# Zokrates/ZoKrates

Hardware: AMD Instinct MI355X
Metric: groth16_proofs_per_sec (higher is better)
Workload: dtype u32

## Files before the change

zokrates_amd/csrc/core.cuh:

```cuda
#pragma once
#include <algorithm>
#include <atomic>
#include <chrono>
#include <cstdio>
#include <memory>
#include <new>
#include <string>
#include <system_error>
#include <thread>
#include <unordered_set>
#include <vector>

#include "../../include/zkhip.h"
#include "devrt.h"
#include "ec.cuh"
#include "kernels_msm.cuh"
#include "kernels_ntt.cuh"

namespace zk {

struct CurveBn254 {
    static constexpr int ID = ZKHIP_CURVE_BN128;
    typedef Fe<Bn254Fr> Fr;
    typedef Fe<Bn254Fq> Fq;
// ... 53 lines not shown
template <class T> static inline T* ptr(const DBuf& b) { return (T*)b.p; }

static inline unsigned blocks_for(u64 n, unsigned threads) { return (unsigned)((n + threads - 1) / threads); }
static inline int ilog2_floor(u64 x) { int l = 0; while (x >>= 1) ++l; return l; }
static inline int ilog2_ceil(u64 x) { int l = 0; while (((u64)1 << l) < x) ++l; return l; }

}

using namespace zk;

struct NttPlanBase {
    int curve, logN;
    virtual ~NttPlanBase() {}
};
struct MsmSort {
    DBuf dig, sorted, cnt, off, cursor, chunk_sum, grand;
    DBuf pairs, ccur, tile_off;
    Event ready = nullptr;
};
struct MsmLane {
    Stream stream = 0;
    bool made = false;
    bool high_priority = false;
    DBuf lane_key, heavy, partial, bucket, rows, cols;
    Event done = nullptr;
    Stream fold_stream = 0;
    bool fold_made = false;
    bool fold_owned = true;
    Event acc_done = nullptr;
    bool lone_launch = false;
    Stream lone_fold_stream = 0;
    bool lone_fold_made = false;
    bool share_cu = false;
};
static constexpr int ZK_NLANES = 5;
static constexpr int ZK_NSLOTS = 4;
struct ProofSlot {
    DBuf scalars, zmont, va, vb, vc, ws1, ws2, zflag;
    MsmSort sorts[3];
    MsmLane lanes[ZK_NLANES];
    void* h_ws = nullptr;
    size_t h_ws_cap = 0;
    Event ev[4] = {nullptr, nullptr, nullptr, nullptr};
    Event acc_b[ZK_NLANES] = {}, acc_e[ZK_NLANES] = {};
    Event ntt_b = nullptr, ntt_e = nullptr;
    Event g1_go = nullptr;
    Event half_ready = nullptr;
// ... 385 lines not shown
static void ntt_kind_b(zkhip_ctx* ctx, NttPlan<C>* pl, typename C::Fr* data, bool inverse, const typename C::Fr* final_post, int nvec = 1,
                       u64 vec_stride = 0, int canon = 0) {
    typedef typename C::Fr Fr;
    if (pl->log3 > 0) {
        ntt_rows<C>(ctx, pl, data, inverse, inverse ? ptr<Fr>(pl->tw2_inv) : ptr<Fr>(pl->tw2_fwd), nvec, vec_stride, 0, nullptr, pl->Nb - 1);
        ntt_mid<C>(ctx, pl, data, inverse, inverse ? ptr<Fr>(pl->tw_inv) : ptr<Fr>(pl->tw_fwd), ~(u64)0, nvec, vec_stride);
        ntt_cols<C>(ctx, pl, data, inverse, final_post, nvec, vec_stride, canon);
    } else if (pl->log1 > 0) {
        ntt_rows<C>(ctx, pl, data, inverse, inverse ? ptr<Fr>(pl->tw_inv) : ptr<Fr>(pl->tw_fwd), nvec, vec_stride);
        ntt_cols<C>(ctx, pl, data, inverse, final_post, nvec, vec_stride, canon);
    } else {
        ntt_rows<C>(ctx, pl, data, inverse, final_post, nvec, vec_stride, canon);
    }
}

struct MsmShape {
    u64 n;
    int c, W;
    u32 K;
    u32 sets;
    u32 levels;
    u32 nkeys;
    u32 Lw, H;
    static constexpr u32 ndig = 2;
    int level_bits() const { return c * (int)sets; }
    bool skip_inf = true;
    u32 nsums() const { return ndig * sets; }
};
static inline int env_int(const char* name, int lo, int hi, int dflt) {
    if (const char* e = getenv(name)) { int v = atoi(e); if (v >= lo && v <= hi) return v; }
    return dflt;
}
static constexpr int MSM_MAX_C = 17;
static constexpr int MSM_AUTO_MAX_C = 17;
static constexpr int MSM_ADHOC_MAX_C = 16;
static constexpr u32 MSM_SORT_MAX_KH = 1u << 15;
static inline MsmShape msm_shape(const zkhip_ctx* ctx, u64 n, int scalar_bits, bool table, int force_c = 0, int force_sets = 0) {
    MsmShape s;
    s.n = n;
    const int lg = ilog2_floor(std::max<u64>(n, 1));
    if (table) {
        const int cmax = std::max(2, std::min(MSM_AUTO_MAX_C, lg + 1));
        const int Wmin = (scalar_bits + 1 + cmax - 1) / cmax;
        s.c = cmax;
        while (s.c > 2 && (scalar_bits + 1 + (s.c - 1) - 1) / (s.c - 1) == Wmin) --s.c;
    } else {
        const int want = std::max(2, std::min(MSM_ADHOC_MAX_C, lg - 5));
// ... 1605 lines not shown
```

zokrates_amd/csrc/devrt.h:

```cpp
#pragma once
#include <algorithm>
#include <atomic>
#include <cstddef>
#include <mutex>
#include <unordered_map>
#include <cstdint>
#include <cstdio>
#include <cstdlib>
#include <cstring>
#include <string>
#include <system_error>
#include <thread>
#include <vector>

#ifdef ZK_EMU
#include "emu.h"
#else
#include <hip/hip_runtime.h>
#endif

namespace zk {

struct DevError {
    std::string msg;
// ... 376 lines not shown
inline bool trace_enabled() {
    static const bool on = getenv("ZKHIP_TRACE") != nullptr;
    return on;
}
inline bool grid_nonempty(const dim3& g) { return g.x != 0 && g.y != 0 && g.z != 0; }
#define ZK_LAUNCH(kernel, grid, block, smem, stream, ...)                                 \
    do {                                                                                  \
        if (!zk::grid_nonempty(dim3(grid))) break;                                        \
        if (zk::trace_enabled()) fprintf(stderr, "[zkhip] launch %s ...", #kernel);       \
        zk::jitter_before(stream);                                                        \
        hipLaunchKernelGGL(kernel, grid, block, smem, stream, __VA_ARGS__);               \
        zk::dev_check_last();                                                             \
        if (zk::trace_enabled()) {                                                        \
            ZK_HIP_CHECK(hipStreamSynchronize(stream));                                   \
            fprintf(stderr, " done\n");                                                   \
        }                                                                                 \
    } while (0)
#define ZK_DYN_SMEM(name) extern __shared__ __attribute__((aligned(16))) unsigned char name[]
#ifndef ZK_WAVE_PRIO
#define ZK_WAVE_PRIO 3
#endif
#define ZK_PRIO_HIGH() __builtin_amdgcn_s_setprio(ZK_WAVE_PRIO)
#define ZK_WAVE_ANY(pred) (__builtin_amdgcn_ballot_w64(pred) != 0)
#ifdef ZK_CHECKED
#define ZK_ASSERT_IDX(cond) do { if (!(cond)) __builtin_trap(); } while (0)
#else
#define ZK_ASSERT_IDX(cond) ((void)0)
#endif

#else

typedef int Stream;
typedef double* Event;
inline int dev_count() { return 1; }
inline void dev_set(int) {}
inline void dev_pci_bus_id(int, char* out, size_t cap) { snprintf(out, cap, "0000:00:00.0"); }
inline void* dev_alloc(size_t bytes) { return aligned_alloc(256, ((bytes ? bytes : 16) + 255) / 256 * 256); }
inline void dev_free(void* p) { free(p); }
inline void* host_alloc_pinned(size_t bytes) { return dev_alloc(bytes); }
inline void host_free_pinned(void* p) { free(p); }
inline void dev_h2d(void* d, const void* h, size_t n, Stream) { memcpy(d, h, n); }
template <class Fill>
inline void dev_h2d_fill(void* d, size_t n, size_t unit, Stream, Fill&& fill, unsigned = 8) {
    const size_t units = n / unit, cut = units / 3 * unit;
    if (cut) fill((char*)d, (size_t)0, cut);
    if (n > cut) fill((char*)d + cut, cut, n - cut);
// ... 7 lines not shown
inline void dev_memset(void* d, int v, size_t n, Stream) { memset(d, v, n); }
inline Stream stream_create() { return 0; }
inline Stream stream_create_high_priority() { return 0; }
inline Stream stream_create_low_priority() { return 0; }
inline void stream_destroy(Stream) {}
inline void stream_sync(Stream) {}
inline void dev_sync_all() {}
inline void dev_mem_info(size_t* free_b, size_t* total_b) { *free_b = *total_b = (size_t)1 << 40; }
inline Event event_create() { return new double(0); }
inline void event_destroy(Event e) { delete e; }
inline void event_record(Event e, Stream) { *e = emu::now_ms(); }
inline void event_sync(Event) {}
inline void stream_wait_event(Stream, Event) {}
inline float event_elapsed_ms(Event a, Event b) { return (float)(*b - *a); }
inline void dev_check_last() {}
struct JitterState { std::atomic<int> max_us{0}; };
inline JitterState& jitter_state() { static JitterState st; return st; }

#define ZK_LAUNCH(kernel, grid, block, smem, stream, ...) \
    emu::launch(dim3(grid), dim3(block), (size_t)(smem), [&]() { kernel(__VA_ARGS__); })
#define ZK_DYN_SMEM(name) unsigned char* name = emu::dyn_smem()
#define ZK_PRIO_HIGH() ((void)0)
#define ZK_WAVE_ANY(pred) (pred)
#ifdef ZK_CHECKED
#define ZK_ASSERT_IDX(cond) do { if (!(cond)) { fprintf(stderr, "ZK_ASSERT_IDX failed: %s (%s:%d)\n", #cond, __FILE__, __LINE__); abort(); } } while (0)
#else
#define ZK_ASSERT_IDX(cond) ((void)0)
#endif

#endif

}
```

zokrates_amd/csrc/group.cuh:

```cuda
#pragma once
#include "core.cuh"
#include "bind.cuh"

namespace zk {

template <class FS>
void points_to_packed(zkhip_ctx* ctx, const Aff<FS>* d_in, void* d_out, u64 n) {
    typedef typename Unsat<FS>::type U;
    ZK_LAUNCH((k_points_to_packed<FS, U>), dim3(blocks_for(n, 256)), dim3(256), 0, ctx->stream, d_in, (AffPacked<U>*)d_out, n);
}

template <class FS>
void msm_table_levels(zkhip_ctx* ctx, void* d_table, u64 count, int c, int W) {
    typedef typename Unsat<FS>::type F;
    if (W <= 1 || count == 0) return;
    const u64 chunk = std::min<u64>(count, std::max<u64>(1024, ((u64)768 << 20) / ((u64)(W - 1) * (sizeof(Xyzz<F>) + sizeof(F)))));
    DBuf tmp, pre;
    tmp.ensure((u64)(W - 1) * chunk * sizeof(Xyzz<F>));
    pre.ensure((u64)(W - 1) * chunk * sizeof(F));
    for (u64 i0 = 0; i0 < count; i0 += chunk) {
        const u64 cnt = std::min(chunk, count - i0);
        ZK_LAUNCH((k_msm_table_levels<F, FS>), dim3(blocks_for(cnt, 256)), dim3(256), 0, ctx->stream, (AffPacked<F>*)d_table, count, i0, cnt, c, W,
                  ptr<Xyzz<F>>(tmp), ptr<F>(pre));
    }
    stream_sync(ctx->stream);
}

template <class FS>
void msm_run_tables(zkhip_ctx* ctx, MsmLane& lane, const MsmSort& so, const void* const* d_tables, int nt, const MsmShape& sh, Xyzz<FS>* d_window_sums,
                    u32 sum_stride, Event ev_begin, Event ev_end, Event accum_after, Xyzz<FS>* h_window_sums) {
    typedef typename Unsat<FS>::type F;
    require(nt >= 1 && nt <= MSM_MAX_TABLES, ZKHIP_ERR_BAD_ARG, "internal: number of tables of one MSM launch");
    MsmTables tables{};
    for (int t = 0; t < nt; ++t) tables.p[t] = d_tables[t];
    Stream s = ctx->serial ? ctx->stream : lane_stream(lane);
    stream_wait_event(s, so.ready);
    const int single = MsmTuning<F>::IS_EXT ? (ctx->msm_g2_waves ? ctx->msm_g2_waves : MsmTuning<F>::SLICE_WPE)
                                            : (ctx->msm_g1_waves ? ctx->msm_g1_waves : MsmTuning<F>::SLICE_WPE);
    const int wpe = ctx->msm_waves ? ctx->msm_waves : (nt > 1 ? std::max(1, (ctx->msm_fused_waves ? ctx->msm_fused_waves : MsmTuning<F>::FUSED_WPE)) : single);
    const u64 machine = ctx->msm_lanes ? (u64)ctx->msm_lanes : (u64)ctx->cus * 4 * 64 * wpe / (nt > 1 && !ctx->msm_waves ? nt : 1);
    const u32 nlanes = (u32)std::max<u64>(1, std::min<u64>(machine, (sh.n * (u64)sh.W + ctx->msm_min_slice - 1) / ctx->msm_min_slice));
    const bool share = lane.share_cu && !ctx->serial;
    lane.share_cu = false;
    const bool lone_launch = lane.lone_launch;
    lane.lone_launch = false;
    const MsmCut cut{nlanes, ctx->msm_min_slice, (u32)std::min<u64>(sh.n * (u64)sh.levels, 0x7fffffffu), share ? 1u : 0u};
    const u64 partial_stride = (u64)sh.nkeys + nlanes;
    lane.heavy.ensure(((size_t)sh.nkeys + 1) * 4);
    lane.lane_key.ensure((size_t)nlanes * 4);
    lane.partial.ensure((size_t)nt * partial_stride * sizeof(Xyzz<F>));
    lane.bucket.ensure((size_t)nt * sh.nkeys * sizeof(Xyzz<F>));
    lane.rows.ensure((size_t)nt * sh.sets * sh.H * sizeof(Xyzz<F>));
    lane.cols.ensure((size_t)nt * sh.sets * sh.Lw * sizeof(Xyzz<F>));
    lds_opt_in(ctx, (const void*)k_msm_fold_rows<F>);
    lds_opt_in(ctx, (const void*)k_msm_fold_cols<F>);
    lds_opt_in(ctx, (const void*)k_msm_fold_final<F, FS>);
    lds_opt_in(ctx, (const void*)k_msm_fold_final_scan<F, FS>);
    const unsigned T = 256;
    ZK_LAUNCH(k_msm_lane_keys, dim3(blocks_for(nlanes, T)), dim3(T), 0, s, ptr<u32>(so.off), sh.nkeys, cut, ptr<u32>(lane.lane_key), ptr<u32>(lane.heavy));
    ZK_LAUNCH(k_msm_find_heavy, dim3(blocks_for(sh.nkeys, T)), dim3(T), 0, s, ptr<u32>(so.off), sh.nkeys, cut, ptr<u32>(lane.heavy) + 1,
              ptr<u32>(lane.heavy));
    if (accum_after && !ctx->serial) stream_wait_event(s, accum_after);
    if (ev_begin) event_record(ev_begin, s);
    const size_t acc_lds = share ? std::max<size_t>(msm_accum_lds_bytes<F>(), (size_t)84 * 1024) : msm_accum_lds_bytes<F>();
    if (ctx->skip_inf_mode == 1 || (ctx->skip_inf_mode == 0 && sh.skip_inf)) {
        if (acc_lds > 64 * 1024) lds_opt_in(ctx, (const void*)k_msm_accum<F, MsmTuning<F>::ACCUM_WPE, true>);
        ZK_LAUNCH((k_msm_accum<F, MsmTuning<F>::ACCUM_WPE, true>), dim3(blocks_for(nlanes, T), nt), dim3(T), acc_lds, s, tables, ptr<u32>(so.off), ptr<u32>(so.sorted),
                  ptr<u32>(lane.lane_key), ptr<Xyzz<F>>(lane.partial), partial_stride, sh.nkeys, cut);
    } else {
        if (acc_lds > 64 * 1024) lds_opt_in(ctx, (const void*)k_msm_accum<F, MsmTuning<F>::ACCUM_WPE, false>);
        ZK_LAUNCH((k_msm_accum<F, MsmTuning<F>::ACCUM_WPE, false>), dim3(blocks_for(nlanes, T), nt), dim3(T), acc_lds, s, tables, ptr<u32>(so.off), ptr<u32>(so.sorted),
                  ptr<u32>(lane.lane_key), ptr<Xyzz<F>>(lane.partial), partial_stride, sh.nkeys, cut);
    }
    if (ev_end) event_record(ev_end, s);
    const bool lone_hop = lone_launch && (lane.lone_fold_made || (MsmTuning<F>::IS_EXT && lane.fold_made));
    if (!ctx->serial && (lone_launch ? lone_hop : (lane.fold_made || ctx->fold_hop == 1 || (ctx->fold_hop == 2 && MsmTuning<F>::IS_EXT)))) {
        event_record(lane.acc_done, s);
        s = (lone_launch && lane.lone_fold_made) ? lane.lone_fold_stream : lane_fold_stream(lane);
        stream_wait_event(s, lane.acc_done);
    }
    if (ctx->heavy_runs) {
        lds_opt_in(ctx, (const void*)k_msm_heavy_reduce<F>);
        const unsigned TH = (unsigned)ctx->heavy_threads;
        ZK_LAUNCH((k_msm_heavy_reduce<F>), dim3(MSM_HEAVY_CHUNKS, nt), dim3(TH), (size_t)TH * sizeof(Xyzz<F>), s, ptr<Xyzz<F>>(lane.partial), partial_stride,
                  ptr<u32>(so.off), sh.nkeys, cut, ptr<u32>(lane.heavy) + 1, ptr<u32>(lane.heavy));
    }
    FoldDigits digs{};
    const u32 widest = std::max(sh.H, sh.Lw);
    if ((ctx->fold_lines == 1 || (ctx->fold_lines == 2 && nt == 1)) && widest <= 256) {
        const unsigned TL = std::max<u32>(64, widest);
        lds_opt_in(ctx, (const void*)k_msm_fold_lines<F>);
        ZK_LAUNCH((k_msm_fold_lines<F>), dim3(widest, sh.sets * 2, nt), dim3(TL), (size_t)TL * sizeof(Xyzz<F>), s, ptr<Xyzz<F>>(lane.partial), partial_stride,
                  ptr<u32>(so.off), sh.nkeys, cut, sh.K, sh.Lw, sh.H, ptr<u32>(lane.heavy) + 1, ptr<u32>(lane.heavy), ctx->heavy_runs ? 1u : 0u,
                  ptr<Xyzz<F>>(lane.rows), ptr<Xyzz<F>>(lane.cols));
    } else {
        ZK_LAUNCH((k_msm_fold_rows<F>), dim3(sh.H, sh.sets, nt), dim3(sh.Lw), (size_t)sh.Lw * sizeof(Xyzz<F>), s, ptr<Xyzz<F>>(lane.partial), partial_stride,
                  ptr<u32>(so.off), sh.nkeys, cut, sh.K, sh.Lw, ptr<u32>(lane.heavy) + 1, ptr<u32>(lane.heavy), ctx->heavy_runs ? 1u : 0u, ptr<Xyzz<F>>(lane.bucket),
                  ptr<Xyzz<F>>(lane.rows));
        const u32 RG = sh.H;
        const u32 HG = std::max<u32>(1, std::min<u32>((u32)ctx->fold_hg, RG)), CW = std::min<u32>(sh.Lw, 256 / HG), NG = sh.H / RG;
        ZK_LAUNCH((k_msm_fold_cols<F>), dim3(sh.Lw / CW, sh.sets * NG, nt), dim3(CW, HG), (size_t)CW * HG * sizeof(Xyzz<F>), s, ptr<Xyzz<F>>(lane.bucket), (u64)sh.K,
                  (u64)sh.nkeys, sh.Lw, sh.H, RG, ptr<Xyzz<F>>(lane.cols));
    }
    digs.d[0] = FoldDigit{lane.cols.p, sh.Lw, 1, 0};
    digs.d[1] = FoldDigit{lane.rows.p, sh.H, 0, (u32)ilog2_floor(sh.Lw)};
    u32 longest = 0;
    for (u32 d = 0; d < sh.ndig; ++d) longest = std::max(longest, digs.d[d].len);
    const unsigned TS = std::max<u32>(64, longest);
    if (ctx->fold_scan && TS <= 256) {
        ZK_LAUNCH((k_msm_fold_final_scan<F, FS>), dim3(sh.sets, nt, sh.ndig), dim3(TS), TS * sizeof(Xyzz<F>), s, digs, d_window_sums, sum_stride);
    } else {
        const unsigned TF = std::max<u32>(64, sh.Lw);
        ZK_LAUNCH((k_msm_fold_final<F, FS>), dim3(sh.sets, nt), dim3(TF), TF * sizeof(Xyzz<F>), s, ptr<Xyzz<F>>(lane.rows), ptr<Xyzz<F>>(lane.cols), sh.Lw,
                  sh.H, d_window_sums, sum_stride);
    }
    if (h_window_sums)
        for (int t = 0; t < nt; ++t)
            dev_d2h_pinned(h_window_sums + (size_t)t * sum_stride, d_window_sums + (size_t)t * sum_stride, (size_t)sh.nsums() * sizeof(Xyzz<FS>), s);
    event_record(lane.done, s);
}
template <class FS>
u64 count_infinite(zkhip_ctx* ctx, const void* d_table, u64 count) {
    typedef typename Unsat<FS>::type F;
    if (!count) return 0;
    DBuf d;
    d.ensure(4);
    dev_memset(d.p, 0, 4, ctx->stream);
    ZK_LAUNCH((k_count_infinite<F>), dim3(blocks_for(count, 256)), dim3(256), 0, ctx->stream, (const AffPacked<F>*)d_table, count, ptr<u32>(d));
    u32 n = 0;
    dev_d2h(&n, d.p, 4, ctx->stream);
    stream_sync(ctx->stream);
    return n;
}
template <class FS>
void mark_finite(zkhip_ctx* ctx, const void* d_table, u64 count, u32* d_bitmap) {
    typedef typename Unsat<FS>::type F;
    ZK_LAUNCH((k_mark_finite<F>), dim3(blocks_for(count, 256)), dim3(256), 0, ctx->stream, (const AffPacked<F>*)d_table, count, d_bitmap);
// ... 73 lines not shown
```

zokrates_amd/csrc/kernels_msm.cuh:

```cuda
#pragma once
#include "devrt.h"
#include "ec.cuh"

namespace zk {

#ifndef ZK_G2_ACCUM_WPE
#define ZK_G2_ACCUM_WPE 2
#endif
#ifndef ZK_G1_FUSED_WPE
#define ZK_G1_FUSED_WPE 6
#endif
#ifndef ZK_G1_SLICE_WPE
#define ZK_G1_SLICE_WPE 4
#endif
#ifndef ZK_G2_SLICE_WPE
#define ZK_G2_SLICE_WPE 4
#endif
#ifndef ZK_G2_COLD_WPE
#define ZK_G2_COLD_WPE 2
#endif
#ifndef ZK_G2_PREFETCH_REGS
#define ZK_G2_PREFETCH_REGS 1
#endif
#ifndef ZK_G2_ZZ_LDS
// ... 467 lines not shown
            sh[threadIdx.x] += t;
            __syncthreads();
        }
        if (i < nchunks) chunk_sum[i] = carry + sh[threadIdx.x] - x;
        __syncthreads();
        if (threadIdx.x == SCAN_THREADS - 1) carry += sh[threadIdx.x];
        __syncthreads();
    }
    if (threadIdx.x == 0) *grand_total = carry;
}
static __global__ void k_scan_add(u32* __restrict__ off, const u32* __restrict__ chunk_sum, u64 total, const u32* __restrict__ grand_total) {
    ZK_PRIO_HIGH();
    u64 i = (u64)blockIdx.x * blockDim.x + threadIdx.x;
    if (i < total) off[i] += chunk_sum[i / SCAN_CHUNK];
    if (i == total) off[total] = *grand_total;
}

struct MsmCut { u32 nlanes, min_slice; u32 table_len; u32 prio; };
static __device__ __forceinline__ u32 msm_slice_len(const u32* __restrict__ off, u32 nkeys, MsmCut cut) {
    const u32 total = off[nkeys];
    const u32 P = (total + cut.nlanes - 1) / cut.nlanes;
    return P > cut.min_slice ? P : cut.min_slice;
}
static __global__ void k_msm_lane_keys(const u32* __restrict__ off, u32 nkeys, MsmCut cut, u32* __restrict__ lane_key, u32* __restrict__ heavy_count) {
    ZK_PRIO_HIGH();
    const u32 g = blockIdx.x * blockDim.x + threadIdx.x;
    if (g == 0) *heavy_count = 0;
    if (g >= cut.nlanes) return;
    const u32 P = msm_slice_len(off, nkeys, cut);
    const u64 pos = (u64)g * P;
    if (pos >= off[nkeys]) { lane_key[g] = nkeys; return; }
    u32 lo = 0, hi = nkeys;
    while (hi - lo > 1) {
        const u32 mid = lo + ((hi - lo) >> 1);
        if (off[mid] <= pos) lo = mid; else hi = mid;
    }
    lane_key[g] = lo;
}
static __global__ void k_msm_find_heavy(const u32* __restrict__ off, u32 nkeys, MsmCut cut, u32* __restrict__ heavy_list,
                                        u32* __restrict__ heavy_count) {
    ZK_PRIO_HIGH();
    const u32 k = blockIdx.x * blockDim.x + threadIdx.x;
    if (k >= nkeys) return;
    const u32 P = msm_slice_len(off, nkeys, cut);
    const u32 b = off[k], e = off[k + 1];
    if (e > b && (e - 1) / P - b / P + 1 > MSM_HEAVY) heavy_list[atomicAdd(heavy_count, 1u)] = k;
}

#if defined(__HIP_DEVICE_COMPILE__)
template <class T>
__device__ __forceinline__ void zk_pin_words(T& obj) {
    u32* w = (u32*)&obj;
    ZK_UNROLL for (unsigned i = 0; i < sizeof(T) / 4; ++i) asm volatile("" : "+v"(w[i]));
}
#define ZK_PIN_WORDS(x) zk_pin_words(x)
#define ZK_LDS_REREAD() asm volatile("" ::: "memory")
#define ZK_OPAQUE(x) asm volatile("" : "+v"(x))
#else
#define ZK_PIN_WORDS(x) ((void)0)
#define ZK_LDS_REREAD() ((void)0)
#define ZK_OPAQUE(x) ((void)0)
#endif
#ifndef ZK_ACCUM_FENCE
#define ZK_ACCUM_FENCE 0
#endif
#ifndef ZK_ACCUM_X_UNREDUCED
#define ZK_ACCUM_X_UNREDUCED 0
#endif
#if defined(__HIP_DEVICE_COMPILE__)
#define ZK_SCHED_FENCE(on) do { if (on) __builtin_amdgcn_sched_barrier(0); } while (0)
#else
#define ZK_SCHED_FENCE(on) ((void)0)
#endif
template <class F, int WPE, bool SKIP_INF>
__global__ void __launch_bounds__(256, WPE) k_msm_accum(MsmTables tables, const u32* __restrict__ off, const u32* __restrict__ sorted,
                                                    const u32* __restrict__ lane_key, Xyzz<F>* __restrict__ partial, u64 partial_stride, u32 nkeys, MsmCut cut) {
    constexpr int NW2 = 2 * AffPacked<F>::NW;
#ifndef ZK_EMU
    if (cut.prio) __builtin_amdgcn_s_setprio(2);
#endif
    const AffPacked<F>* __restrict__ bases = (const AffPacked<F>*)tables.p[blockIdx.y];
    partial += (u64)blockIdx.y * partial_stride;
    const u32 g = blockIdx.x * blockDim.x + threadIdx.x;
    if (g >= cut.nlanes) return;
    u32 cur = lane_key[g];
    if (cur >= nkeys) return;
    const u32 total = off[nkeys];
    const u32 P = msm_slice_len(off, nkeys, cut);
    const u32 p0 = g * P;
    const u32 p1 = total - p0 > P ? p0 + P : total;
    u32 end = off[cur + 1], nend = off[cur + 2 < nkeys ? cur + 2 : nkeys];
    ZK_ASSERT_IDX((u64)g * P < total && off[cur] <= p0 && p0 < end && (u64)nkeys + cut.nlanes <= partial_stride);
    constexpr bool ZZ_LDS = MsmTuning<F>::ZZ_IN_LDS, XY_LDS = MsmTuning<F>::XY_IN_LDS;
    constexpr int FW = (int)(sizeof(F) / 4);
    ZK_DYN_SMEM(acc_smem);
    u32* const acc_lds = (u32*)acc_smem;
    constexpr int XY_BASE = ZZ_LDS ? 2 : 0;
    F rxy[2] = {F::zero(), F::zero()}, rzz[2] = {F::zero(), F::zero()};
    auto lds_get = [&](int slot) -> F {
        F r;
        u32* wv = (u32*)&r;
        ZK_LDS_REREAD();
        ZK_UNROLL for (int q = 0; q < FW; ++q) wv[q] = acc_lds[(slot * FW + q) * 256 + threadIdx.x];
        return r;
    };
    auto lds_put = [&](int slot, const F& v) {
        const u32* wv = (const u32*)&v;
        ZK_UNROLL for (int q = 0; q < FW; ++q) acc_lds[(slot * FW + q) * 256 + threadIdx.x] = wv[q];
    };
    auto get_zz = [&](int which) -> F { return ZZ_LDS ? lds_get(which) : rzz[which]; };
    auto put_zz = [&](int which, const F& v) { if (ZZ_LDS) lds_put(which, v); else rzz[which] = v; };
// ... 110 lines not shown
__device__ __forceinline__ void block_tree_sum_reg(Xyzz<F>* sh, Xyzz<F>& v, unsigned width) {
    __syncthreads();
    for (unsigned st = width >> 1; st > 0; st >>= 1) {
        if (threadIdx.x < st) {
            xyzz_add_from(v, &sh[threadIdx.x + st]);
            if (st > 1) sh[threadIdx.x] = v;
        }
        __syncthreads();
    }
}

template <class F>
__device__ __forceinline__ Xyzz<F> xyzz_mul_small(const Xyzz<F>& p, u32 k) {
    Xyzz<F> r = Xyzz<F>::inf();
    if (k == 0 || p.is_inf()) return r;
    for (int i = 31 - __clz(k); i >= 0; --i) {
        r = xyzz_dbl_inl(r);
        if ((k >> i) & 1) xyzz_add_acc(r, p);
    }
    return r;
}

static constexpr u32 MSM_HEAVY_CHUNKS = 64;
struct HeavyRun {
    u32 g0, g1, len;
};
static __device__ __forceinline__ HeavyRun msm_heavy_run(const u32* __restrict__ off, u32 key, u32 P) {
    HeavyRun r;
    r.g0 = off[key] / P;
    r.g1 = (off[key + 1] - 1) / P;
    r.len = (r.g1 - r.g0 + MSM_HEAVY_CHUNKS) / MSM_HEAVY_CHUNKS;
    return r;
}
template <class F>
__global__ void __launch_bounds__(256, MsmTuning<F>::COLD_WPE) k_msm_heavy_reduce(Xyzz<F>* partial, u64 partial_stride, const u32* __restrict__ off, u32 nkeys, MsmCut cut,
                                                                                  const u32* __restrict__ heavy_list, const u32* __restrict__ heavy_count) {
    ZK_PRIO_HIGH();
    const u32 nh = *heavy_count;
    if (nh == 0) return;
    ZK_DYN_SMEM(smem);
    Xyzz<F>* sh = (Xyzz<F>*)smem;
    partial += (u64)blockIdx.y * partial_stride;
    const u32 P = msm_slice_len(off, nkeys, cut), lo = threadIdx.x;
    for (u32 h = 0; h < nh; ++h) {
        const u32 hk = heavy_list[h];
        const HeavyRun r = msm_heavy_run(off, hk, P);
        const u32 b = r.g0 + blockIdx.x * r.len;
        if (b > r.g1 || r.len == 1) continue;
        const u32 e = b + r.len - 1 < r.g1 ? b + r.len - 1 : r.g1;
        Xyzz<F> s = Xyzz<F>::inf();
        for (u32 g = b + lo; g <= e; g += blockDim.x) xyzz_add_from(s, &partial[(u64)hk + g]);
        sh[lo] = s;
        block_tree_sum<F>(sh);
        if (lo == 0) partial[(u64)hk + b] = sh[0];
        __syncthreads();
    }
}
template <class F>
__global__ void __launch_bounds__(256, MsmTuning<F>::COLD_WPE) k_msm_fold_rows(Xyzz<F>* partial, u64 partial_stride, const u32* __restrict__ off, u32 nkeys, MsmCut cut, u32 K, u32 Lw,
                                                        const u32* __restrict__ heavy_list, const u32* __restrict__ heavy_count, u32 heavy_runs,
                                                        Xyzz<F>* __restrict__ bucket, Xyzz<F>* __restrict__ rows) {
    ZK_PRIO_HIGH();
    ZK_DYN_SMEM(smem);
    Xyzz<F>* sh = (Xyzz<F>*)smem;
    partial += (u64)blockIdx.z * partial_stride;
    bucket += (u64)blockIdx.z * nkeys;
    rows += (u64)blockIdx.z * gridDim.y * gridDim.x;
    const u32 j = blockIdx.y, hi = blockIdx.x, lo = threadIdx.x;
    const u32 P = msm_slice_len(off, nkeys, cut);
    const u32 row0 = j * K + hi * Lw;
    const u32 nh = *heavy_count;
    for (u32 h = 0; h < nh; ++h) {
        const u32 hk = heavy_list[h];
        if (hk - row0 >= Lw) continue;
        const HeavyRun r = msm_heavy_run(off, hk, P);
        const u32 g0 = r.g0, g1 = r.g1, step = heavy_runs ? r.len : 1;
        Xyzz<F> s = Xyzz<F>::inf();
        for (u64 g = g0 + (u64)lo * step; g <= g1; g += (u64)blockDim.x * step) xyzz_add_from(s, &partial[(u64)hk + g]);
        sh[lo] = s;
        block_tree_sum<F>(sh);
        if (lo == 0) partial[(u64)hk + g0] = sh[0];
        __syncthreads();
    }
    const u32 key = row0 + lo;
    ZK_ASSERT_IDX(key < nkeys && (u64)key + (off[key + 1] ? (off[key + 1] - 1) / P : 0) < partial_stride);
    Xyzz<F> v = msm_bucket_sum<F>(partial, off, key, P);
    bucket[key] = v;
    sh[lo] = v;
    block_tree_sum<F>(sh);
    if (lo == 0) rows[(u64)j * gridDim.x + hi] = sh[0];
}
template <class F>
__global__ void __launch_bounds__(256, MsmTuning<F>::COLD_WPE) k_msm_fold_lines(const Xyzz<F>* __restrict__ partial, u64 partial_stride, const u32* __restrict__ off, u32 nkeys,
                                                                                MsmCut cut, u32 K, u32 Lw, u32 H, const u32* __restrict__ heavy_list,
                                                                                const u32* __restrict__ heavy_count, u32 heavy_runs, Xyzz<F>* __restrict__ rows,
                                                                                Xyzz<F>* __restrict__ cols) {
    ZK_PRIO_HIGH();
    ZK_DYN_SMEM(smem);
    Xyzz<F>* sh = (Xyzz<F>*)smem;
    const u32 sets = gridDim.y >> 1, j = blockIdx.y >> 1, dir = blockIdx.y & 1u, line = blockIdx.x, t = threadIdx.x;
    const u32 len = dir ? H : Lw, nlines = dir ? Lw : H;
    if (line >= nlines) return;
    partial += (u64)blockIdx.z * partial_stride;
    const u32 P = msm_slice_len(off, nkeys, cut);
    const u32 set0 = j * K;
    const bool live = t < len;
    const u32 key = set0 + (dir ? t * Lw + line : line * Lw + t);
    Xyzz<F> v = Xyzz<F>::inf();
    bool have = !live;
    const u32 nh = *heavy_count;
    for (u32 h = 0; h < nh; ++h) {
        const u32 hk = heavy_list[h];
        const u32 rel = hk - set0;
        if (rel >= K || (dir ? rel % Lw : rel / Lw) != line) continue;
        const HeavyRun r = msm_heavy_run(off, hk, P);
        const u32 step = heavy_runs ? r.len : 1;
        Xyzz<F> s = Xyzz<F>::inf();
        for (u64 g = r.g0 + (u64)t * step; g <= r.g1; g += (u64)blockDim.x * step) xyzz_add_from(s, &partial[(u64)hk + g]);
        sh[t] = s;
        block_tree_sum_reg<F>(sh, s, blockDim.x);
        if (t == 0) sh[0] = s;
        __syncthreads();
        if (live && key == hk) { v = sh[0]; have = true; }
        __syncthreads();
    }
    if (!have) {
        ZK_ASSERT_IDX(key < nkeys && (u64)key + (off[key + 1] ? (off[key + 1] - 1) / P : 0) < partial_stride);
        v = msm_bucket_sum<F>(partial, off, key, P);
    }
    sh[t] = v;
    block_tree_sum_reg<F>(sh, v, blockDim.x);
    if (t == 0) (dir ? cols : rows)[((u64)blockIdx.z * sets + j) * nlines + line] = v;
}
template <class F>
__global__ void __launch_bounds__(256, MsmTuning<F>::COLD_WPE) k_msm_fold_cols(const Xyzz<F>* __restrict__ src, u64 set_stride, u64 msm_stride, u32 Lw, u32 H, u32 RG,
                                                                               Xyzz<F>* __restrict__ dst) {
    ZK_PRIO_HIGH();
    ZK_DYN_SMEM(smem);
    Xyzz<F>* sh = (Xyzz<F>*)smem;
    const u32 NG = H / RG, sets = gridDim.y / NG;
    const u32 j = blockIdx.y / NG, g = blockIdx.y % NG;
    const u32 lo = blockIdx.x * blockDim.x + threadIdx.x, hg = threadIdx.y, HG = blockDim.y;
    src += (u64)blockIdx.z * msm_stride + (u64)j * set_stride + (u64)g * RG * Lw;
    dst += (((u64)blockIdx.z * sets + j) * NG + g) * Lw;
    Xyzz<F> s = Xyzz<F>::inf();
    for (u32 hi = hg; hi < RG; hi += HG) xyzz_add_from(s, &src[(u64)hi * Lw + lo]);
    sh[hg * blockDim.x + threadIdx.x] = s;
    __syncthreads();
    for (unsigned st = HG >> 1; st > 0; st >>= 1) {
        if (hg < st) {
            Xyzz<F> a = sh[hg * blockDim.x + threadIdx.x];
            xyzz_add_from(a, &sh[(hg + st) * blockDim.x + threadIdx.x]);
            sh[hg * blockDim.x + threadIdx.x] = a;
        }
        __syncthreads();
    }
    if (hg == 0) dst[lo] = sh[threadIdx.x];
}
template <class F, class FS>
__global__ void __launch_bounds__(256, MsmTuning<F>::COLD_WPE) k_msm_fold_final(const Xyzz<F>* __restrict__ rows, const Xyzz<F>* __restrict__ cols, u32 Lw, u32 H,
                                                         Xyzz<FS>* __restrict__ window_sum, u32 sum_stride) {
    ZK_PRIO_HIGH();
    ZK_DYN_SMEM(smem);
    Xyzz<F>* sh = (Xyzz<F>*)smem;
    const u32 j = blockIdx.x, t = threadIdx.x;
    rows += (u64)blockIdx.y * gridDim.x * H;
    cols += (u64)blockIdx.y * gridDim.x * Lw;
    window_sum += (u64)blockIdx.y * sum_stride;
    Xyzz<F> term = Xyzz<F>::inf();
    for (u32 hi = t; hi < H; hi += blockDim.x) xyzz_add_acc(term, xyzz_mul_small(rows[(u64)j * H + hi], hi));
    sh[t] = term;
    block_tree_sum<F>(sh);
    Xyzz<F> hi_sum = sh[0];
    __syncthreads();
    term = Xyzz<F>::inf();
    for (u32 lo = t; lo < Lw; lo += blockDim.x) xyzz_add_acc(term, xyzz_mul_small(cols[(u64)j * Lw + lo], lo + 1));
    sh[t] = term;
    block_tree_sum<F>(sh);
    if (t == 0) {
        for (u32 q = Lw; q > 1; q >>= 1) hi_sum = xyzz_dbl_inl(hi_sum);
        Xyzz<F> r = sh[0];
        xyzz_add_acc(r, hi_sum);
        window_sum[2 * j] = xyzz_to_sat<FS>(r);
        window_sum[2 * j + 1] = Xyzz<FS>::inf();
    }
}

struct FoldDigit {
    const void* src;
    u32 len;
    u32 plus_one;
    u32 dbl;
};
struct FoldDigits { FoldDigit d[2]; };
template <class F, class FS>
__global__ void __launch_bounds__(256, MsmTuning<F>::COLD_WPE) k_msm_fold_final_scan(FoldDigits digs, Xyzz<FS>* __restrict__ window_sum, u32 sum_stride) {
    ZK_PRIO_HIGH();
    ZK_DYN_SMEM(smem);
    Xyzz<F>* sh = (Xyzz<F>*)smem;
    const u32 j = blockIdx.x, t = threadIdx.x, nd = gridDim.z;
    const FoldDigit dg = blockIdx.z == 0 ? digs.d[0] : digs.d[1];
    const u32 seglen = dg.len;
    const Xyzz<F>* src = (const Xyzz<F>*)dg.src + ((u64)blockIdx.y * gridDim.x + j) * seglen;
    window_sum += (u64)blockIdx.y * sum_stride;
    const bool live = t < seglen;
    Xyzz<F> v = Xyzz<F>::inf();
    if (live) v = src[t];
    sh[t] = v;
    __syncthreads();
    for (u32 d = 1; d < seglen; d <<= 1) {
        const bool has = live && t + d < seglen;
        if (has) xyzz_add_from(v, &sh[t + d]);
        __syncthreads();
        if (has) sh[t] = v;
        __syncthreads();
    }
    if (!dg.plus_one && t == 0) {
        v = Xyzz<F>::inf();
        sh[0] = v;
    }
    block_tree_sum_reg<F>(sh, v, seglen);
    if (t == 0) {
        Xyzz<F> r = v;
        for (u32 q = 0; q < dg.dbl; ++q) r = xyzz_dbl_inl(r);
        window_sum[nd * j + blockIdx.z] = xyzz_to_sat<FS>(r);
    }
}

template <class F, class FS>
__global__ void __launch_bounds__(256) k_msm_table_levels(AffPacked<F>* __restrict__ tbl, u64 stride, u64 i0, u64 cnt, int c, int W,
                                                           Xyzz<F>* __restrict__ tmp, F* __restrict__ pre) {
    const u64 i = (u64)blockIdx.x * blockDim.x + threadIdx.x;
    if (i >= cnt) return;
    u32 w[2 * AffPacked<F>::NW];
    aff_load_words<F>(tbl, i0 + i, w);
    Xyzz<F> P = Xyzz<F>::from_affine(aff_unpack<F>(w));
    F acc = F::one();
    for (int j = 1; j < W; ++j) {
        for (int b = 0; b < c; ++b) P = xyzz_dbl_inl(P);
        tmp[(u64)(j - 1) * cnt + i] = P;
        if (!P.is_inf()) {
            pre[(u64)(j - 1) * cnt + i] = acc;
            acc = ec_mul(acc, P.zzz);
        }
    }
    F inv = ec_inv(acc);
    for (int j = W - 1; j >= 1; --j) {
        const Xyzz<F> Q = tmp[(u64)(j - 1) * cnt + i];
        Aff<F> a = Aff<F>::inf();
// ... 63 lines not shown
```

Baseline: 114.7.

## Fuse MSM lane-key/heavy-list setup into accum and finalize folds via last-block tickets

Removes the separate lane-key and heavy-bucket kernels by computing each lane's first key with a binary search and building the heavy list inside the accumulate kernel. When fold_scan is enabled, the final window-sum scan is folded into the rows and cols fold kernels: the last block per set, found with an atomic ticket and agent-scope fences, performs the digit scan. The heavy counter is now reset by whichever fold kernel runs last instead of by a prelude kernel. This cuts several small kernel launches per MSM but adds atomics, fences and a serialized tail block, and depends on the counters being zeroed correctly.

```diff
diff --git a/zokrates_amd/csrc/core.cuh b/zokrates_amd/csrc/core.cuh
--- a/zokrates_amd/csrc/core.cuh
+++ b/zokrates_amd/csrc/core.cuh
@@ -99,7 +99,7 @@
     Stream stream = 0;
     bool made = false;
     bool high_priority = false;
-    DBuf lane_key, heavy, partial, bucket, rows, cols;
+    DBuf heavy, ticket, partial, bucket, rows, cols;
     Event done = nullptr;
     Stream fold_stream = 0;
     bool fold_made = false;
@@ -531,7 +531,7 @@
     u32 levels;
     u32 nkeys;
     u32 Lw, H;
-    static constexpr u32 ndig = 2;
+    static constexpr u32 ndig = MSM_FOLD_DIGITS;
     int level_bits() const { return c * (int)sets; }
     bool skip_inf = true;
     u32 nsums() const { return ndig * sets; }
diff --git a/zokrates_amd/csrc/devrt.h b/zokrates_amd/csrc/devrt.h
--- a/zokrates_amd/csrc/devrt.h
+++ b/zokrates_amd/csrc/devrt.h
@@ -422,6 +422,11 @@
 #endif
 #define ZK_PRIO_HIGH() __builtin_amdgcn_s_setprio(ZK_WAVE_PRIO)
 #define ZK_WAVE_ANY(pred) (__builtin_amdgcn_ballot_w64(pred) != 0)
+#define ZK_DRAIN_STORES() asm volatile("s_waitcnt vmcnt(0)" ::: "memory")
+#define ZK_AGENT_RELEASE() do { __builtin_amdgcn_fence(__ATOMIC_RELEASE, "agent"); asm volatile("s_waitcnt vmcnt(0)" ::: "memory"); } while (0)
+#define ZK_AGENT_ACQUIRE() do { __builtin_amdgcn_fence(__ATOMIC_ACQUIRE, "agent"); asm volatile("s_waitcnt vmcnt(0)" ::: "memory"); } while (0)
+#define ZK_TICKET_TAKE(p) __hip_atomic_fetch_add((p), 1u, __ATOMIC_RELAXED, __HIP_MEMORY_SCOPE_AGENT)
+#define ZK_TICKET_RESET(p) __hip_atomic_store((p), 0u, __ATOMIC_RELAXED, __HIP_MEMORY_SCOPE_AGENT)
 #ifdef ZK_CHECKED
 #define ZK_ASSERT_IDX(cond) do { if (!(cond)) __builtin_trap(); } while (0)
 #else
@@ -475,6 +480,11 @@
 #define ZK_DYN_SMEM(name) unsigned char* name = emu::dyn_smem()
 #define ZK_PRIO_HIGH() ((void)0)
 #define ZK_WAVE_ANY(pred) (pred)
+#define ZK_DRAIN_STORES() ((void)0)
+#define ZK_AGENT_RELEASE() ((void)0)
+#define ZK_AGENT_ACQUIRE() ((void)0)
+#define ZK_TICKET_TAKE(p) atomicAdd((p), 1u)
+#define ZK_TICKET_RESET(p) (*(p) = 0u)
 #ifdef ZK_CHECKED
 #define ZK_ASSERT_IDX(cond) do { if (!(cond)) { fprintf(stderr, "ZK_ASSERT_IDX failed: %s (%s:%d)\n", #cond, __FILE__, __LINE__); abort(); } } while (0)
 #else
diff --git a/zokrates_amd/csrc/group.cuh b/zokrates_amd/csrc/group.cuh
--- a/zokrates_amd/csrc/group.cuh
+++ b/zokrates_amd/csrc/group.cuh
@@ -46,31 +46,34 @@
     lane.lone_launch = false;
     const MsmCut cut{nlanes, ctx->msm_min_slice, (u32)std::min<u64>(sh.n * (u64)sh.levels, 0x7fffffffu), share ? 1u : 0u};
     const u64 partial_stride = (u64)sh.nkeys + nlanes;
-    lane.heavy.ensure(((size_t)sh.nkeys + 1) * 4);
-    lane.lane_key.ensure((size_t)nlanes * 4);
+    auto ensure_zeroed = [&](DBuf& b, size_t bytes, size_t zero_bytes) {
+        const size_t before = b.cap;
+        b.ensure(bytes);
+        if (b.cap != before) dev_memset(b.p, 0, zero_bytes, s);
+    };
+    ensure_zeroed(lane.heavy, ((size_t)sh.nkeys + 4) * 4, 16);
+    const size_t ticket_bytes = ((size_t)2 * nt * sh.sets * 4 + 15) / 16 * 16;
+    ensure_zeroed(lane.ticket, ticket_bytes, ticket_bytes);
     lane.partial.ensure((size_t)nt * partial_stride * sizeof(Xyzz<F>));
     lane.bucket.ensure((size_t)nt * sh.nkeys * sizeof(Xyzz<F>));
     lane.rows.ensure((size_t)nt * sh.sets * sh.H * sizeof(Xyzz<F>));
     lane.cols.ensure((size_t)nt * sh.sets * sh.Lw * sizeof(Xyzz<F>));
-    lds_opt_in(ctx, (const void*)k_msm_fold_rows<F>);
-    lds_opt_in(ctx, (const void*)k_msm_fold_cols<F>);
+    lds_opt_in(ctx, (const void*)k_msm_fold_rows<F, FS>);
+    lds_opt_in(ctx, (const void*)k_msm_fold_cols<F, FS>);
     lds_opt_in(ctx, (const void*)k_msm_fold_final<F, FS>);
     lds_opt_in(ctx, (const void*)k_msm_fold_final_scan<F, FS>);
     const unsigned T = 256;
-    ZK_LAUNCH(k_msm_lane_keys, dim3(blocks_for(nlanes, T)), dim3(T), 0, s, ptr<u32>(so.off), sh.nkeys, cut, ptr<u32>(lane.lane_key), ptr<u32>(lane.heavy));
-    ZK_LAUNCH(k_msm_find_heavy, dim3(blocks_for(sh.nkeys, T)), dim3(T), 0, s, ptr<u32>(so.off), sh.nkeys, cut, ptr<u32>(lane.heavy) + 1,
-              ptr<u32>(lane.heavy));
     if (accum_after && !ctx->serial) stream_wait_event(s, accum_after);
     if (ev_begin) event_record(ev_begin, s);
     const size_t acc_lds = share ? std::max<size_t>(msm_accum_lds_bytes<F>(), (size_t)84 * 1024) : msm_accum_lds_bytes<F>();
     if (ctx->skip_inf_mode == 1 || (ctx->skip_inf_mode == 0 && sh.skip_inf)) {
         if (acc_lds > 64 * 1024) lds_opt_in(ctx, (const void*)k_msm_accum<F, MsmTuning<F>::ACCUM_WPE, true>);
         ZK_LAUNCH((k_msm_accum<F, MsmTuning<F>::ACCUM_WPE, true>), dim3(blocks_for(nlanes, T), nt), dim3(T), acc_lds, s, tables, ptr<u32>(so.off), ptr<u32>(so.sorted),
-                  ptr<u32>(lane.lane_key), ptr<Xyzz<F>>(lane.partial), partial_stride, sh.nkeys, cut);
+                  ptr<u32>(lane.heavy) + 1, ptr<u32>(lane.heavy), ptr<Xyzz<F>>(lane.partial), partial_stride, sh.nkeys, cut);
     } else {
         if (acc_lds > 64 * 1024) lds_opt_in(ctx, (const void*)k_msm_accum<F, MsmTuning<F>::ACCUM_WPE, false>);
         ZK_LAUNCH((k_msm_accum<F, MsmTuning<F>::ACCUM_WPE, false>), dim3(blocks_for(nlanes, T), nt), dim3(T), acc_lds, s, tables, ptr<u32>(so.off), ptr<u32>(so.sorted),
-                  ptr<u32>(lane.lane_key), ptr<Xyzz<F>>(lane.partial), partial_stride, sh.nkeys, cut);
+                  ptr<u32>(lane.heavy) + 1, ptr<u32>(lane.heavy), ptr<Xyzz<F>>(lane.partial), partial_stride, sh.nkeys, cut);
     }
     if (ev_end) event_record(ev_end, s);
     const bool lone_hop = lone_launch && (lane.lone_fold_made || (MsmTuning<F>::IS_EXT && lane.fold_made));
@@ -87,32 +90,35 @@
     }
     FoldDigits digs{};
     const u32 widest = std::max(sh.H, sh.Lw);
-    if ((ctx->fold_lines == 1 || (ctx->fold_lines == 2 && nt == 1)) && widest <= 256) {
+    const bool lines = (ctx->fold_lines == 1 || (ctx->fold_lines == 2 && nt == 1)) && widest <= 256;
+    const unsigned TS = std::max<u32>(64, widest);
+    const bool scan = ctx->fold_scan && TS <= 256;
+    u32* const tickets = scan && !lines ? ptr<u32>(lane.ticket) : nullptr;
+    if (lines) {
         const unsigned TL = std::max<u32>(64, widest);
         lds_opt_in(ctx, (const void*)k_msm_fold_lines<F>);
         ZK_LAUNCH((k_msm_fold_lines<F>), dim3(widest, sh.sets * 2, nt), dim3(TL), (size_t)TL * sizeof(Xyzz<F>), s, ptr<Xyzz<F>>(lane.partial), partial_stride,
                   ptr<u32>(so.off), sh.nkeys, cut, sh.K, sh.Lw, sh.H, ptr<u32>(lane.heavy) + 1, ptr<u32>(lane.heavy), ctx->heavy_runs ? 1u : 0u,
                   ptr<Xyzz<F>>(lane.rows), ptr<Xyzz<F>>(lane.cols));
     } else {
-        ZK_LAUNCH((k_msm_fold_rows<F>), dim3(sh.H, sh.sets, nt), dim3(sh.Lw), (size_t)sh.Lw * sizeof(Xyzz<F>), s, ptr<Xyzz<F>>(lane.partial), partial_stride,
+        ZK_LAUNCH((k_msm_fold_rows<F, FS>), dim3(sh.H, sh.sets, nt), dim3(sh.Lw), (size_t)sh.Lw * sizeof(Xyzz<F>), s, ptr<Xyzz<F>>(lane.partial), partial_stride,
                   ptr<u32>(so.off), sh.nkeys, cut, sh.K, sh.Lw, ptr<u32>(lane.heavy) + 1, ptr<u32>(lane.heavy), ctx->heavy_runs ? 1u : 0u, ptr<Xyzz<F>>(lane.bucket),
-                  ptr<Xyzz<F>>(lane.rows));
+                  ptr<Xyzz<F>>(lane.rows), tickets, d_window_sums, sum_stride, (u32)ilog2_floor(sh.Lw));
         const u32 RG = sh.H;
         const u32 HG = std::max<u32>(1, std::min<u32>((u32)ctx->fold_hg, RG)), CW = std::min<u32>(sh.Lw, 256 / HG), NG = sh.H / RG;
-        ZK_LAUNCH((k_msm_fold_cols<F>), dim3(sh.Lw / CW, sh.sets * NG, nt), dim3(CW, HG), (size_t)CW * HG * sizeof(Xyzz<F>), s, ptr<Xyzz<F>>(lane.bucket), (u64)sh.K,
-                  (u64)sh.nkeys, sh.Lw, sh.H, RG, ptr<Xyzz<F>>(lane.cols));
+        ZK_LAUNCH((k_msm_fold_cols<F, FS>), dim3(sh.Lw / CW, sh.sets * NG, nt), dim3(CW, HG), (size_t)CW * HG * sizeof(Xyzz<F>), s, ptr<Xyzz<F>>(lane.bucket), (u64)sh.K,
+                  (u64)sh.nkeys, sh.Lw, sh.H, RG, ptr<Xyzz<F>>(lane.cols), tickets ? tickets + (size_t)nt * sh.sets : nullptr, d_window_sums, sum_stride,
+                  ptr<u32>(lane.heavy));
     }
     digs.d[0] = FoldDigit{lane.cols.p, sh.Lw, 1, 0};
     digs.d[1] = FoldDigit{lane.rows.p, sh.H, 0, (u32)ilog2_floor(sh.Lw)};
-    u32 longest = 0;
-    for (u32 d = 0; d < sh.ndig; ++d) longest = std::max(longest, digs.d[d].len);
-    const unsigned TS = std::max<u32>(64, longest);
-    if (ctx->fold_scan && TS <= 256) {
-        ZK_LAUNCH((k_msm_fold_final_scan<F, FS>), dim3(sh.sets, nt, sh.ndig), dim3(TS), TS * sizeof(Xyzz<F>), s, digs, d_window_sums, sum_stride);
+    if (tickets) {
+    } else if (scan) {
+        ZK_LAUNCH((k_msm_fold_final_scan<F, FS>), dim3(sh.sets, nt, sh.ndig), dim3(TS), TS * sizeof(Xyzz<F>), s, digs, d_window_sums, sum_stride, ptr<u32>(lane.heavy));
     } else {
         const unsigned TF = std::max<u32>(64, sh.Lw);
         ZK_LAUNCH((k_msm_fold_final<F, FS>), dim3(sh.sets, nt), dim3(TF), TF * sizeof(Xyzz<F>), s, ptr<Xyzz<F>>(lane.rows), ptr<Xyzz<F>>(lane.cols), sh.Lw,
-                  sh.H, d_window_sums, sum_stride);
+                  sh.H, d_window_sums, sum_stride, ptr<u32>(lane.heavy));
     }
     if (h_window_sums)
         for (int t = 0; t < nt; ++t)
diff --git a/zokrates_amd/csrc/kernels_msm.cuh b/zokrates_amd/csrc/kernels_msm.cuh
--- a/zokrates_amd/csrc/kernels_msm.cuh
+++ b/zokrates_amd/csrc/kernels_msm.cuh
@@ -513,29 +513,22 @@
     const u32 P = (total + cut.nlanes - 1) / cut.nlanes;
     return P > cut.min_slice ? P : cut.min_slice;
 }
-static __global__ void k_msm_lane_keys(const u32* __restrict__ off, u32 nkeys, MsmCut cut, u32* __restrict__ lane_key, u32* __restrict__ heavy_count) {
-    ZK_PRIO_HIGH();
-    const u32 g = blockIdx.x * blockDim.x + threadIdx.x;
-    if (g == 0) *heavy_count = 0;
-    if (g >= cut.nlanes) return;
-    const u32 P = msm_slice_len(off, nkeys, cut);
+static __device__ __forceinline__ u32 msm_first_key(const u32* __restrict__ off, u32 nkeys, u32 total, u32 P, u32 g) {
     const u64 pos = (u64)g * P;
-    if (pos >= off[nkeys]) { lane_key[g] = nkeys; return; }
+    if (pos >= total) return nkeys;
     u32 lo = 0, hi = nkeys;
     while (hi - lo > 1) {
         const u32 mid = lo + ((hi - lo) >> 1);
         if (off[mid] <= pos) lo = mid; else hi = mid;
     }
-    lane_key[g] = lo;
-}
-static __global__ void k_msm_find_heavy(const u32* __restrict__ off, u32 nkeys, MsmCut cut, u32* __restrict__ heavy_list,
-                                        u32* __restrict__ heavy_count) {
-    ZK_PRIO_HIGH();
-    const u32 k = blockIdx.x * blockDim.x + threadIdx.x;
-    if (k >= nkeys) return;
-    const u32 P = msm_slice_len(off, nkeys, cut);
-    const u32 b = off[k], e = off[k + 1];
-    if (e > b && (e - 1) / P - b / P + 1 > MSM_HEAVY) heavy_list[atomicAdd(heavy_count, 1u)] = k;
+    return lo;
+}
+static __device__ __forceinline__ void msm_list_heavy(const u32* __restrict__ off, u32 nkeys, u32 P, u32 g, u32 width, u32* __restrict__ heavy_list,
+                                                      u32* __restrict__ heavy_count) {
+    for (u32 k = g; k < nkeys; k += width) {
+        const u32 b = off[k], e = off[k + 1];
+        if (e - b > P && (e - 1) / P - b / P + 1 > MSM_HEAVY) heavy_list[atomicAdd(heavy_count, 1u)] = k;
+    }
 }
 
 #if defined(__HIP_DEVICE_COMPILE__)
@@ -565,7 +558,8 @@
 #endif
 template <class F, int WPE, bool SKIP_INF>
 __global__ void __launch_bounds__(256, WPE) k_msm_accum(MsmTables tables, const u32* __restrict__ off, const u32* __restrict__ sorted,
-                                                    const u32* __restrict__ lane_key, Xyzz<F>* __restrict__ partial, u64 partial_stride, u32 nkeys, MsmCut cut) {
+                                                    u32* __restrict__ heavy_list, u32* __restrict__ heavy_count, Xyzz<F>* __restrict__ partial, u64 partial_stride,
+                                                    u32 nkeys, MsmCut cut) {
     constexpr int NW2 = 2 * AffPacked<F>::NW;
 #ifndef ZK_EMU
     if (cut.prio) __builtin_amdgcn_s_setprio(2);
@@ -573,11 +567,12 @@
     const AffPacked<F>* __restrict__ bases = (const AffPacked<F>*)tables.p[blockIdx.y];
     partial += (u64)blockIdx.y * partial_stride;
     const u32 g = blockIdx.x * blockDim.x + threadIdx.x;
-    if (g >= cut.nlanes) return;
-    u32 cur = lane_key[g];
-    if (cur >= nkeys) return;
     const u32 total = off[nkeys];
     const u32 P = msm_slice_len(off, nkeys, cut);
+    if (blockIdx.y == 0) msm_list_heavy(off, nkeys, P, g, gridDim.x * blockDim.x, heavy_list, heavy_count);
+    if (g >= cut.nlanes) return;
+    u32 cur = msm_first_key(off, nkeys, total, P, g);
+    if (cur >= nkeys) return;
     const u32 p0 = g * P;
     const u32 p1 = total - p0 > P ? p0 + P : total;
     u32 end = off[cur + 1], nend = off[cur + 2 < nkeys ? cur + 2 : nkeys];
@@ -734,6 +729,7 @@
 }
 
 static constexpr u32 MSM_HEAVY_CHUNKS = 64;
+static constexpr u32 MSM_FOLD_DIGITS = 2;
 struct HeavyRun {
     u32 g0, g1, len;
 };
@@ -768,10 +764,30 @@
         __syncthreads();
     }
 }
-template <class F>
+static __device__ __forceinline__ bool fold_hand_off(void* sh, u32* ticket, u32 ntickets, bool leader) {
+    ZK_DRAIN_STORES();
+    __syncthreads();
+    volatile u32* const flag = (volatile u32*)sh;
+    if (leader) {
+        ZK_AGENT_RELEASE();
+        const bool last = ZK_TICKET_TAKE(ticket) == ntickets - 1;
+        if (last) {
+            ZK_TICKET_RESET(ticket);
+            ZK_AGENT_ACQUIRE();
+        }
+        *flag = last ? 1u : 0u;
+    }
+    __syncthreads();
+    const bool last = *flag != 0;
+    __syncthreads();
+    return last;
+}
+template <class F, class FS>
+__device__ __forceinline__ void msm_digit_scan(Xyzz<F>* sh, const Xyzz<F>* src, u32 seglen, u32 plus_one, u32 dbl, u32 t, Xyzz<FS>* out);
+template <class F, class FS>
 __global__ void __launch_bounds__(256, MsmTuning<F>::COLD_WPE) k_msm_fold_rows(Xyzz<F>* partial, u64 partial_stride, const u32* __restrict__ off, u32 nkeys, MsmCut cut, u32 K, u32 Lw,
                                                         const u32* __restrict__ heavy_list, const u32* __restrict__ heavy_count, u32 heavy_runs,
-                                                        Xyzz<F>* __restrict__ bucket, Xyzz<F>* __restrict__ rows) {
+                                                        Xyzz<F>* __restrict__ bucket, Xyzz<F>* rows, u32* ticket, Xyzz<FS>* __restrict__ window_sum, u32 sum_stride, u32 dbl) {
     ZK_PRIO_HIGH();
     ZK_DYN_SMEM(smem);
     Xyzz<F>* sh = (Xyzz<F>*)smem;
@@ -801,6 +817,9 @@
     sh[lo] = v;
     block_tree_sum<F>(sh);
     if (lo == 0) rows[(u64)j * gridDim.x + hi] = sh[0];
+    if (!ticket) return;
+    if (!fold_hand_off(sh, ticket + blockIdx.z * gridDim.y + j, gridDim.x, lo == 0)) return;
+    msm_digit_scan<F, FS>(sh, rows + (u64)j * gridDim.x, gridDim.x, 0, dbl, lo, window_sum + (u64)blockIdx.z * sum_stride + MSM_FOLD_DIGITS * j + 1);
 }
 template <class F>
 __global__ void __launch_bounds__(256, MsmTuning<F>::COLD_WPE) k_msm_fold_lines(const Xyzz<F>* __restrict__ partial, u64 partial_stride, const u32* __restrict__ off, u32 nkeys,
@@ -844,12 +863,14 @@
     block_tree_sum_reg<F>(sh, v, blockDim.x);
     if (t == 0) (dir ? cols : rows)[((u64)blockIdx.z * sets + j) * nlines + line] = v;
 }
-template <class F>
+template <class F, class FS>
 __global__ void __launch_bounds__(256, MsmTuning<F>::COLD_WPE) k_msm_fold_cols(const Xyzz<F>* __restrict__ src, u64 set_stride, u64 msm_stride, u32 Lw, u32 H, u32 RG,
-                                                                               Xyzz<F>* __restrict__ dst) {
+                                                                               Xyzz<F>* dst, u32* ticket, Xyzz<FS>* __restrict__ window_sum, u32 sum_stride,
+                                                                               u32* __restrict__ heavy_count) {
     ZK_PRIO_HIGH();
     ZK_DYN_SMEM(smem);
     Xyzz<F>* sh = (Xyzz<F>*)smem;
+    if (ticket && (threadIdx.x | threadIdx.y | blockIdx.x | blockIdx.y | blockIdx.z) == 0) *heavy_count = 0;
     const u32 NG = H / RG, sets = gridDim.y / NG;
     const u32 j = blockIdx.y / NG, g = blockIdx.y % NG;
     const u32 lo = blockIdx.x * blockDim.x + threadIdx.x, hg = threadIdx.y, HG = blockDim.y;
@@ -868,14 +889,19 @@
         __syncthreads();
     }
     if (hg == 0) dst[lo] = sh[threadIdx.x];
+    if (!ticket) return;
+    const u32 t = hg * blockDim.x + threadIdx.x;
+    if (!fold_hand_off(sh, ticket + blockIdx.z * sets + j, gridDim.x, t == 0)) return;
+    msm_digit_scan<F, FS>(sh, dst, Lw, 1, 0, t, window_sum + (u64)blockIdx.z * sum_stride + MSM_FOLD_DIGITS * j);
 }
 template <class F, class FS>
 __global__ void __launch_bounds__(256, MsmTuning<F>::COLD_WPE) k_msm_fold_final(const Xyzz<F>* __restrict__ rows, const Xyzz<F>* __restrict__ cols, u32 Lw, u32 H,
-                                                         Xyzz<FS>* __restrict__ window_sum, u32 sum_stride) {
+                                                         Xyzz<FS>* __restrict__ window_sum, u32 sum_stride, u32* __restrict__ heavy_count) {
     ZK_PRIO_HIGH();
     ZK_DYN_SMEM(smem);
     Xyzz<F>* sh = (Xyzz<F>*)smem;
     const u32 j = blockIdx.x, t = threadIdx.x;
+    if (t == 0 && (blockIdx.x | blockIdx.y) == 0) *heavy_count = 0;
     rows += (u64)blockIdx.y * gridDim.x * H;
     cols += (u64)blockIdx.y * gridDim.x * Lw;
     window_sum += (u64)blockIdx.y * sum_stride;
@@ -906,15 +932,7 @@
 };
 struct FoldDigits { FoldDigit d[2]; };
 template <class F, class FS>
-__global__ void __launch_bounds__(256, MsmTuning<F>::COLD_WPE) k_msm_fold_final_scan(FoldDigits digs, Xyzz<FS>* __restrict__ window_sum, u32 sum_stride) {
-    ZK_PRIO_HIGH();
-    ZK_DYN_SMEM(smem);
-    Xyzz<F>* sh = (Xyzz<F>*)smem;
-    const u32 j = blockIdx.x, t = threadIdx.x, nd = gridDim.z;
-    const FoldDigit dg = blockIdx.z == 0 ? digs.d[0] : digs.d[1];
-    const u32 seglen = dg.len;
-    const Xyzz<F>* src = (const Xyzz<F>*)dg.src + ((u64)blockIdx.y * gridDim.x + j) * seglen;
-    window_sum += (u64)blockIdx.y * sum_stride;
+__device__ __forceinline__ void msm_digit_scan(Xyzz<F>* sh, const Xyzz<F>* src, u32 seglen, u32 plus_one, u32 dbl, u32 t, Xyzz<FS>* out) {
     const bool live = t < seglen;
     Xyzz<F> v = Xyzz<F>::inf();
     if (live) v = src[t];
@@ -927,16 +945,35 @@
         if (has) sh[t] = v;
         __syncthreads();
     }
-    if (!dg.plus_one && t == 0) {
+    if (!plus_one && t == 0) {
         v = Xyzz<F>::inf();
         sh[0] = v;
     }
-    block_tree_sum_reg<F>(sh, v, seglen);
+    __syncthreads();
+    for (u32 st = seglen >> 1; st > 0; st >>= 1) {
+        if (t < st) {
+            xyzz_add_from(v, &sh[t + st]);
+            if (st > 1) sh[t] = v;
+        }
+        __syncthreads();
+    }
     if (t == 0) {
         Xyzz<F> r = v;
-        for (u32 q = 0; q < dg.dbl; ++q) r = xyzz_dbl_inl(r);
-        window_sum[nd * j + blockIdx.z] = xyzz_to_sat<FS>(r);
-    }
+        for (u32 q = 0; q < dbl; ++q) r = xyzz_dbl_inl(r);
+        *out = xyzz_to_sat<FS>(r);
+    }
+}
+template <class F, class FS>
+__global__ void __launch_bounds__(256, MsmTuning<F>::COLD_WPE) k_msm_fold_final_scan(FoldDigits digs, Xyzz<FS>* __restrict__ window_sum, u32 sum_stride,
+                                                                                     u32* __restrict__ heavy_count) {
+    ZK_PRIO_HIGH();
+    ZK_DYN_SMEM(smem);
+    Xyzz<F>* sh = (Xyzz<F>*)smem;
+    const u32 j = blockIdx.x, t = threadIdx.x, nd = gridDim.z;
+    if (t == 0 && (blockIdx.x | blockIdx.y | blockIdx.z) == 0) *heavy_count = 0;
+    const FoldDigit dg = blockIdx.z == 0 ? digs.d[0] : digs.d[1];
+    const Xyzz<F>* src = (const Xyzz<F>*)dg.src + ((u64)blockIdx.y * gridDim.x + j) * dg.len;
+    msm_digit_scan<F, FS>(sh, src, dg.len, dg.plus_one, dg.dbl, t, window_sum + (u64)blockIdx.y * sum_stride + nd * j + blockIdx.z);
 }
 
 template <class F, class FS>
```

Measured after the change: 109.9. 4.1% lower.
